# aaletov/open-pcc-metric

Measured on AMD Instinct MI355X. Metric: Mpoints/s for symmetric D1+D2 PSNR, N_ref=N_deg=1M, higher is better.
Workload: dtype f64

## Files before the change

### open_pcc_metric_amd/csrc/pccm_brick.h

```cpp
#pragma once
#include "pccm_grid.h"

namespace pccm {

constexpr int kBXMax = 64;
constexpr int kLcsPitch = kBXMax + 3;
typedef float v2f __attribute__((ext_vector_type(2)));
constexpr float kBigF = 3.0e38f;
constexpr int kExtra = 21;
constexpr float kFar = 1.0e18f;

struct BrickParams {
    int bx;
    int nbx, nby, nbz;
    int64_t per_job;
    uint32_t total;
    int cap;
    unsigned long long *stamps;
    float h32[3], face_lo[3], face_hi[3];
    float org32x, invh32x;
};

__device__ __forceinline__ float face32(float q, int c, int dim, float h, float flo, float fhi)
{
    const float cf = (float)c;
    const float lo = q - __builtin_fmaf(cf, h, flo), hi = __builtin_fmaf(cf, h, fhi) - q;
    const float a = c >= 2 ? lo : INFINITY, b = c <= dim - 3 ? hi : INFINITY;
    return a < b ? a : b;
}

__device__ __forceinline__ float umin_f(float a, float b)
{
    const uint32_t x = __float_as_uint(a), y = __float_as_uint(b);
    return __uint_as_float(x < y ? x : y);
}

constexpr int kPlaneSmall = 2176, kPlaneMid = 3008, kPlaneLarge = 3584;

}
```

### open_pcc_metric_amd/csrc/pccm_brick.hip

```cpp
#include "pccm_brick.h"
#include "pccm_tail_wave.h"

namespace pccm {

#define BRICK_STAMP(k)                                                                       \
    do {                                                                                     \
        if (STAMP) {                                                                         \
            const unsigned long long now_ = __builtin_amdgcn_s_memtime();                    \
            t_sum[k] += now_ - t_last;         \
            t_last = now_;                                                                   \
        }                                                                                    \
    } while (0)

__device__ __forceinline__ void load_normal(const NNOut &o, int row, double &a, double &b, double &c)
{
    if (o.nrm32) {
        const float4 t = o.nrm32[row];
        a = (double)t.x; b = (double)t.y; c = (double)t.z;
    } else {
        const double *np = o.nrm + 3 * (int64_t)row;
        a = np[0]; b = np[1]; c = np[2];
    }
}

__device__ __forceinline__ void tail_append(const QueryJobs &jobs, const QueryJob &J, const float4 q)
{
    const uint32_t pos = atomicAdd(&J.counters[1], 1u);
    reinterpret_cast<float4 *>(J.tail)[pos] = q;
    if (J.blk_cnt) {
        const uint32_t blk = (uint32_t)(__float_as_int(q.w) - (int)J.row_base) >> kTailBlockShift;
        const uint32_t slot = atomicAdd(&J.blk_cnt[blk], 1u);
        if (slot < (uint32_t)kTailBlockCap) J.blk_list[(size_t)blk * kTailBlockCap + slot] = q;
        else if (jobs.err) atomicOr(jobs.err, kErrTailFiled);
        const float nan = __int_as_float(0x7fc00000);
        store_result_rec(J.out, __float_as_int(q.w), nan, nan, nan, -1);
    }
}

template <bool SELF, int BY, int BZ, bool STAMP, int ABL, bool N32, int PL>
__device__ __forceinline__ void brick_body(const QueryJobs &jobs, const GridGeom &g, const BrickParams &bp, const uint32_t vblock)
{
    if (ABL & 32) return;
    const int NT = (int)blockDim.x;
    unsigned long long t_last = STAMP ? __builtin_amdgcn_s_memtime() : 0ull;
    const unsigned long long t_start = t_last;
    unsigned long long t_sum[6] = {0, 0, 0, 0, 0, 0};
    constexpr int kNRow = BY * BZ;
    constexpr int kNRun = (BY + 2) * (BZ + 2);
    static_assert(kNRun <= 64 && kNRow <= 64, "one wave scans the run / row lengths");
    extern __shared__ __attribute__((aligned(16))) float s_pl[];
    static_assert(8 * PL * 4 / 2 < 65536 && 12 * PL < 65536, "plane offsets are 16-bit immediates");
    __shared__ uint16_t s_lcs[kNRun * kLcsPitch];
    __shared__ uint32_t s_g0[kNRun], s_len[kNRun], s_base[kNRun + 1], s_qg0[kNRow], s_qoff[kNRow + 1];
    float *const s_x = s_pl, *const s_y = s_pl + PL, *const s_z = s_pl + 2 * PL, *const s_r = s_pl + 3 * PL;
    const uint32_t lds0 = (uint32_t)(uintptr_t)s_x;
    const int tid = threadIdx.x, lane = tid & 63;
    const int w = __builtin_amdgcn_readfirstlane(tid >> 6);
    const uint32_t nblk = bp.total, xcd = vblock & 7u, slot = vblock >> 3;
    const uint32_t bq = nblk >> 3, br = nblk & 7u;
    int64_t vb = (int64_t)(xcd < br ? xcd * (bq + 1) : br * (bq + 1) + (xcd - br) * bq) + slot;
    const int jb = (jobs.njobs > 1 && vb >= bp.per_job) ? 1 : 0;
    if (jb) vb -= bp.per_job;
    if (vb >= bp.per_job) return;
    const QueryJob &J = jobs.j[jb];
    const int dimx = g.dim[0], dimy = g.dim[1], dimz = g.dim[2];
    const uint32_t vbu = (uint32_t)vb;
    const uint32_t t_xy = vbu / (uint32_t)bp.nbx;
    const uint32_t t_z = t_xy / (uint32_t)bp.nby;
    const int ibx = (int)(vbu - t_xy * (uint32_t)bp.nbx), iby = (int)(t_xy - t_z * (uint32_t)bp.nby), ibz = (int)t_z;
    const int bx0 = ibx * bp.bx, bx1 = min(bx0 + bp.bx, dimx);
    const int by0 = iby * BY, bz0 = ibz * BZ;
    const int sx0 = max(bx0 - 1, 0), sx1 = min(bx1 + 1, dimx);
    const int ncs = sx1 - sx0;
    const uint32_t *__restrict__ cs = J.cs;
    const uint32_t *__restrict__ qcs = J.qcs;
    const Rec32 *__restrict__ srecs = (const Rec32 *)J.srecs;
    const Rec32 *__restrict__ qbase = (const Rec32 *)J.qbase;

    if (w == 0) {
        uint32_t len = 0, g0 = 0;
        if (lane < kNRun) {
            const int y = by0 - 1 + lane % (BY + 2), z = bz0 - 1 + lane / (BY + 2);
            if (y >= 0 && y < dimy && z >= 0 && z < dimz) {
                const uint32_t rowbase = ((uint32_t)z * dimy + y) * dimx;
                g0 = cs[rowbase + sx0];
                len = cs[rowbase + sx1] - g0;
            }
            s_g0[lane] = g0;
            s_len[lane] = len;
        }
        const uint32_t plen = (len + 1u) & ~1u;
        uint32_t inc = plen;
#pragma unroll
        for (int off = 1; off < 64; off <<= 1) {
            const uint32_t o = __shfl_up(inc, off);
            if (lane >= off) inc += o;
        }
        if (lane < kNRun) s_base[lane] = inc - plen;
        if (lane == kNRun - 1) s_base[kNRun] = inc;
    } else if (w == 1) {
        uint32_t len = 0, q0 = 0;
        if (lane < kNRow) {
            const int y = by0 + lane % BY, z = bz0 + lane / BY;
            if (y < dimy && z < dimz) {
                const uint32_t rowbase = ((uint32_t)z * dimy + y) * dimx;
                q0 = qcs[rowbase + bx0];
                len = qcs[rowbase + bx1] - q0;
            }
            s_qg0[lane] = q0;
        }
        uint32_t inc = len;
#pragma unroll
        for (int off = 1; off < 64; off <<= 1) {
            const uint32_t o = __shfl_up(inc, off);
            if (lane >= off) inc += o;
        }
        if (lane < kNRow) s_qoff[lane] = inc - len;
        if (lane == kNRow - 1) s_qoff[kNRow] = inc;
    }
    __syncthreads();
    BRICK_STAMP(0);
    if (ABL & 16) return;
    const uint32_t T = s_base[kNRun], NQ = s_qoff[kNRow];
    if (NQ == 0) return;

    auto query_row = [&](uint32_t qi) {
        int r = 0;
#pragma unroll
        for (int k = 1; k < kNRow; ++k) r += (qi >= s_qoff[k]) ? 1 : 0;
        return r;
    };
    auto load_query = [&](uint32_t qi, int r) {
        return *reinterpret_cast<const float4 *>(&qbase[s_qg0[r] + (qi - s_qoff[r])]);
    };

    if (T > (uint32_t)bp.cap) {
        for (uint32_t qi = tid; qi < NQ; qi += NT) {
            const float4 q = load_query(qi, query_row(qi));
            tail_append(jobs, J, q);
        }
        return;
    }

    uint32_t qi = tid;
    bool have = qi < NQ;
    int rn = 0;
    float4 qn = make_float4(0.f, 0.f, 0.f, 0.f);
    if (have) rn = query_row(qi);

    const NNOut &out = J.out;
    const bool fuse = out.nrm != nullptr;
    const bool fuse_row = fuse && out.normal_mode == PCCM_NORMAL_ROW;
    double n0 = 0.0, n1 = 0.0, n2 = 0.0;
    float4 nraw = make_float4(0.f, 0.f, 0.f, 0.f);
    const bool defer = out.layout == 1;
    auto gather_row_normal = [&](int row, bool on) {
        if (defer) return;
        if (N32) {
            const float4 *src = on ? out.nrm32 + row : reinterpret_cast<const float4 *>(qbase);
            nraw = *src;
        } else if (on) {
            const double *np = out.nrm + 3 * (int64_t)row;
            n0 = np[0]; n1 = np[1]; n2 = np[2];
        }
    };
    {
        const int nw = NT >> 6;
        for (int r0 = w; r0 < kNRun; r0 += 3 * nw) {
            float4 rec[3], rex;
            uint32_t rb[3], rl[3], rg[3];
#pragma unroll
            for (int u = 0; u < 3; ++u) {
                const int r = r0 + u * nw;
                rb[u] = rl[u] = rg[u] = 0u;
                if (r < kNRun) {
                    rb[u] = (uint32_t)__builtin_amdgcn_readfirstlane((int)s_base[r]);
                    rl[u] = (uint32_t)__builtin_amdgcn_readfirstlane((int)s_len[r]);
                    rg[u] = (uint32_t)__builtin_amdgcn_readfirstlane((int)s_g0[r]);
                }
                rec[u] = make_float4(kFar, kFar, kFar, __int_as_float(-1));
                if (!(ABL & 2) && (uint32_t)lane < rl[u]) rec[u] = *reinterpret_cast<const float4 *>(&srecs[rg[u] + (uint32_t)lane]);
            }
            const int xu = lane / kExtra;
            const uint32_t xp = 64u + (uint32_t)(lane - xu * kExtra);
            const uint32_t xb = xu == 0 ? rb[0] : xu == 1 ? rb[1] : rb[2];
            const uint32_t xl = xu == 0 ? rl[0] : xu == 1 ? rl[1] : xu == 2 ? rl[2] : 0u;
            const uint32_t xg = xu == 0 ? rg[0] : xu == 1 ? rg[1] : rg[2];
            rex = make_float4(kFar, kFar, kFar, __int_as_float(-1));
            if (!(ABL & 2) && xp < xl) rex = *reinterpret_cast<const float4 *>(&srecs[xg + xp]);
            uint32_t v[3][2];
            bool in[3];
#pragma unroll
            for (int u = 0; u < 3; ++u) {
                const int r = r0 + u * nw;
                v[u][0] = v[u][1] = 0u;
                in[u] = false;
                if (r < kNRun) {
                    const int y = by0 - 1 + r % (BY + 2), z = bz0 - 1 + r / (BY + 2);
                    in[u] = y >= 0 && y < dimy && z >= 0 && z < dimz;
                    if (in[u] && !(ABL & 8)) {
                        const uint32_t *src = cs + ((uint32_t)z * dimy + y) * dimx + sx0;
                        if (lane <= ncs) v[u][0] = src[lane];
                        if (lane + 64 <= ncs) v[u][1] = src[lane + 64];
                    }
                }
            }
            if (have && r0 == w) qn = load_query(qi, rn);
#pragma unroll
            for (int u = 0; u < 3; ++u) {
                const uint32_t plen = (rl[u] + 1u) & ~1u;
                if ((uint32_t)lane < plen) {
                    const uint32_t f = rb[u] + (uint32_t)lane;
                    s_x[f] = rec[u].x;
                    s_y[f] = rec[u].y;
                    s_z[f] = rec[u].z;
                    s_r[f] = rec[u].w;
                }
            }
            if (xp < ((xl + 1u) & ~1u)) {
                const uint32_t f = xb + xp;
                s_x[f] = rex.x;
                s_y[f] = rex.y;
                s_z[f] = rex.z;
                s_r[f] = rex.w;
            }
#pragma unroll
            for (int u = 0; u < 3; ++u) {
                const uint32_t plen = (rl[u] + 1u) & ~1u;
                for (uint32_t p = (uint32_t)lane + 64u + (uint32_t)kExtra; p < plen; p += 64u) {
                    float4 t = make_float4(kFar, kFar, kFar, __int_as_float(-1));
                    if (!(ABL & 2) && p < rl[u]) t = *reinterpret_cast<const float4 *>(&srecs[rg[u] + p]);
                    const uint32_t f = rb[u] + p;
                    s_x[f] = t.x;
                    s_y[f] = t.y;
                    s_z[f] = t.z;
                    s_r[f] = t.w;
                }
            }
#pragma unroll
            for (int u = 0; u < 3; ++u) {
                const int r = r0 + u * nw;
                if (r < kNRun) {
                    const uint32_t base = lds0 + 4u * rb[u], rebase = base - 4u * rg[u];
                    if (lane <= ncs) s_lcs[r * kLcsPitch + lane] = (uint16_t)(in[u] ? 4u * v[u][0] + rebase : base);
                    if (lane + 64 <= ncs) s_lcs[r * kLcsPitch + lane + 64] = (uint16_t)(in[u] ? 4u * v[u][1] + rebase : base);
                }
            }
        }
        __builtin_amdgcn_sched_barrier(0);
        gather_row_normal(__float_as_int(qn.w), have && fuse_row);
    }
    BRICK_STAMP(1);
    __syncthreads();
    BRICK_STAMP(2);

    int q_iter = 0;
    while (have) {
        const float4 q = qn;
        const int r = rn;
        const int qrow = __float_as_int(q.w);
        const uint32_t qnext = qi + NT;
        const bool hn = qnext < NQ;
        const double qx = (double)q.x, qy = (double)q.y, qz = (double)q.z;
        const int ly = r % BY, lz = r / BY;
        const int cx = min(max((int)floorf((q.x - bp.org32x) * bp.invh32x), bx0), bx1 - 1);
        const int cy = by0 + ly, cz = bz0 + lz;
        const int ja = max(cx - 1, 0) - sx0, jb2 = min(cx + 2, dimx) - sx0;
        float best = kBigF, second = kBigF;
        uint32_t bestpos = 0xffffffffu;
        const v2f qxx = {q.x, q.x}, qyy = {q.y, q.y}, qzz = {q.z, q.z};
#pragma unroll
        for (int dz = 0; dz < 3; ++dz) {
#pragma unroll
            for (int dy = 0; dy < 3; ++dy) {
                const int run = (lz + dz) * (BY + 2) + (ly + dy);
                const uint32_t fsb = s_lcs[run * kLcsPitch + ja], feb = s_lcs[run * kLcsPitch + jb2];
                if constexpr (ABL != 0) {
                for (uint32_t a = fsb & ~7u, ae = (ABL & 1) ? (fsb < feb ? a + 8u : a) : feb; a < ae; a += 8u) {
                    v2f px, py, pz;
                    asm volatile("ds_read_b64 %0, %3\n\tds_read_b64 %1, %3 offset:%4\n\tds_read_b64 %2, %3 offset:%5\n\ts_waitcnt lgkmcnt(0)"
                                 : "=&v"(px), "=&v"(py), "=&v"(pz)
                                 : "v"(a), "n"(4 * PL), "n"(8 * PL)
                                 : "memory");
                    const v2f dx = qxx - px, dy = qyy - py, dz = qzz - pz;
                    v2f dd = dx * dx;
                    dd = __builtin_elementwise_fma(dy, dy, dd);
                    dd = __builtin_elementwise_fma(dz, dz, dd);
                    const float lo = umin_f(dd.x, dd.y);
                    bestpos = __float_as_uint(lo) < __float_as_uint(best) ? a + 8u : bestpos;
                    second = __builtin_amdgcn_fmed3f(best, second, lo);
                    best = umin_f(best, lo);
                }
                } else {
                    uint32_t a = fsb & ~7u;
                    const uint32_t ae = feb;
                    v2f px, py, pz, pr;
                    if (SELF)
                        asm volatile("ds_read_b64 %0, %4\n\tds_read_b64 %1, %4 offset:%5\n\tds_read_b64 %2, %4 offset:%6\n\tds_read_b64 %3, %4 offset:%7"
                                     : "=v"(px), "=v"(py), "=v"(pz), "=v"(pr) : "v"(a), "n"(4 * PL), "n"(8 * PL), "n"(12 * PL) : "memory");
                    else
                        asm volatile("ds_read_b64 %0, %3\n\tds_read_b64 %1, %3 offset:%4\n\tds_read_b64 %2, %3 offset:%5"
                                     : "=v"(px), "=v"(py), "=v"(pz) : "v"(a), "n"(4 * PL), "n"(8 * PL) : "memory");
                    while (a < ae) {
                        if (SELF) asm volatile("s_waitcnt lgkmcnt(0)" : "+v"(px), "+v"(py), "+v"(pz), "+v"(pr) : : "memory");
                        else asm volatile("s_waitcnt lgkmcnt(0)" : "+v"(px), "+v"(py), "+v"(pz) : : "memory");
                        v2f dx = qxx - px, dy = qyy - py, dz = qzz - pz;
                        uint32_t k0 = 0u, k1 = 0u;
                        if (SELF) {
                            k0 = __float_as_int(pr.x) == qrow ? __float_as_uint(kBigF) : 0u;
                            k1 = __float_as_int(pr.y) == qrow ? __float_as_uint(kBigF) : 0u;
                            asm volatile("" : "+v"(k0), "+v"(k1));
                        }
                        asm volatile("" : "+v"(dx), "+v"(dy), "+v"(dz));
                        a += 8u;
                        if (SELF)
                            asm volatile("ds_read_b64 %0, %4\n\tds_read_b64 %1, %4 offset:%5\n\tds_read_b64 %2, %4 offset:%6\n\tds_read_b64 %3, %4 offset:%7"
                                         : "+v"(px), "+v"(py), "+v"(pz), "+v"(pr) : "v"(a), "n"(4 * PL), "n"(8 * PL), "n"(12 * PL) : "memory");
                        else
                            asm volatile("ds_read_b64 %0, %3\n\tds_read_b64 %1, %3 offset:%4\n\tds_read_b64 %2, %3 offset:%5"
                                         : "+v"(px), "+v"(py), "+v"(pz) : "v"(a), "n"(4 * PL), "n"(8 * PL) : "memory");
                        v2f dd = dx * dx;
                        dd = __builtin_elementwise_fma(dy, dy, dd);
                        dd = __builtin_elementwise_fma(dz, dz, dd);
                        float d0 = dd.x, d1 = dd.y;
                        if (SELF) {
                            d0 = __uint_as_float(max(__float_as_uint(d0), k0));
                            d1 = __uint_as_float(max(__float_as_uint(d1), k1));
                        }
                        const float lo = umin_f(d0, d1);
                        bestpos = __float_as_uint(lo) < __float_as_uint(best) ? a : bestpos;
                        second = __builtin_amdgcn_fmed3f(best, second, lo);
                        best = umin_f(best, lo);
                    }
                    if (SELF) asm volatile("s_waitcnt lgkmcnt(0)" : "+v"(px), "+v"(py), "+v"(pz), "+v"(pr) : : "memory");
                    else asm volatile("s_waitcnt lgkmcnt(0)" : "+v"(px), "+v"(py), "+v"(pz) : : "memory");
                }
            }
        }
        BRICK_STAMP(5);
        const float thr = __builtin_fmaf(best, 1.0f + 0x1.0p-18f, 2.0e-36f);
        bool settled = false;
        if (ABL & 4) {
            if (best < 0.0f) store_result(out, qrow, 0.0, 0.0, 0);
            settled = true;
        } else if (bestpos != 0xffffffffu && best < 1.0e30f && second > thr) {
            uint32_t f = (bestpos - 8u - lds0) >> 2;
            float partner;
            {
                const v2f px = *reinterpret_cast<const v2f *>(s_x + f), py = *reinterpret_cast<const v2f *>(s_y + f),
                          pz = *reinterpret_cast<const v2f *>(s_z + f);
                const v2f dx = qxx - px, dy = qyy - py, dz = qzz - pz;
                v2f dd = dx * dx;
                dd = __builtin_elementwise_fma(dy, dy, dd);
                dd = __builtin_elementwise_fma(dz, dz, dd);
                float d0 = dd.x, d1 = dd.y;
                if (SELF) {
                    d0 = (__float_as_int(s_r[f]) == qrow) ? kBigF : d0;
                    d1 = (__float_as_int(s_r[f + 1]) == qrow) ? kBigF : d1;
                }
                const bool first = d0 == best;
                partner = first ? d1 : d0;
                f += first ? 0u : 1u;
            }
            float L = face32(q.x, cx, dimx, bp.h32[0], bp.face_lo[0], bp.face_hi[0]);
            L = fminf(L, face32(q.y, cy, dimy, bp.h32[1], bp.face_lo[1], bp.face_hi[1]));
            L = fminf(L, face32(q.z, cz, dimz, bp.h32[2], bp.face_lo[2], bp.face_hi[2]));
            settled = partner > thr && L > 0.0f && best * 1.00001f < L * L * 0.99999f;
            const float wx = s_x[f], wy = s_y[f], wz = s_z[f];
            const int wrow = __float_as_int(s_r[f]);
            if (settled && defer) {
                store_result_rec(out, qrow, wx, wy, wz, wrow);
            } else if (settled) {
                const double rx = (double)wx, ry = (double)wy, rz = (double)wz;
                const double d64 = gdist64(qx, qy, qz, rx, ry, rz);
                double p = 0.0;
                if (fuse) {
                    double e0 = N32 ? (double)nraw.x : n0, e1 = N32 ? (double)nraw.y : n1, e2 = N32 ? (double)nraw.z : n2;
                    if (!fuse_row) {
                        load_normal(out, wrow, e0, e1, e2);
                    }
                    const double ex = __dsub_rn(qx, rx), ey = __dsub_rn(qy, ry), ez = __dsub_rn(qz, rz);
                    p = __dmul_rn(ex, e0);
                    p = __fma_rn(ey, e1, p);
                    p = __fma_rn(ez, e2, p);
                }
                store_result(out, qrow, d64, p, wrow);
            }
        }
        if (!settled) tail_append(jobs, J, q);
        if (hn) {
            rn = query_row(qnext);
            qn = load_query(qnext, rn);
            gather_row_normal(__float_as_int(qn.w), fuse_row);
        }
        qi = qnext;
        have = hn;
        if (STAMP) {
            BRICK_STAMP(q_iter == 0 ? 3 : 4);
            ++q_iter;
        }
    }
    if (STAMP && lane == 0) {
        unsigned long long *slot = bp.stamps + ((size_t)blockIdx.x * (NT >> 6) + w) * 8;
#pragma unroll
        for (int k = 0; k < 6; ++k) slot[k] = t_sum[k];
        slot[6] = t_start;
        slot[7] = __builtin_amdgcn_s_memtime();
    }
}

template <bool SELF, int BY, int BZ, int PL, bool STAMP = false, int ABL = 0, bool N32 = true>
__global__ __launch_bounds__(1024, 8) void k_brick_query(QueryJobs jobs, GridGeom g, BrickParams bp)
{
    brick_body<SELF, BY, BZ, STAMP, ABL, N32, PL>(jobs, g, bp, blockIdx.x);
}

template <int BY, int BZ, int PL>
__global__ __launch_bounds__(1024) void k_brick_query_free(QueryJobs jobs, GridGeom g, BrickParams bp)
{
    brick_body<false, BY, BZ, false, 0, false, PL>(jobs, g, bp, blockIdx.x);
}

struct BrickShape {
    int by, bz, nt;
};

static BrickShape brick_shape()
{
    static const BrickShape s = [] {
        BrickShape v = {4, 2, 0};
        const char *e = getenv("PCCM_BRICK");
        if (e) {
            int a = 0, b = 0, c = 0;
            const int got = sscanf(e, "%d,%d,%d", &a, &b, &c);
            if (got >= 2) v = {a, b, got == 3 ? c : 0};
        }
        return v;
    }();
    return s;
}

template <int BY, int BZ, int PL>
static void launch_plane(pccm_ctx *ctx, const QueryJobs &jobs, const GridGeom &g, bool self, BrickParams bp, double density_q, int force_nt)
{
    constexpr int kStatic = (BY + 2) * (BZ + 2) * (kLcsPitch * 2 + 12) + (BY * BZ) * 8 + 64;
    static_assert(4 * PL * (int)sizeof(float) + kStatic <= 64 * 1024, "static + dynamic LDS of one workgroup stay under 64 KB");
    const double eq = (double)(BY * BZ) * bp.bx * density_q;
    int nt = ((int)(eq + 2.5 * sqrt(eq)) + 63) / 64 * 64;
    const size_t lds = (size_t)4 * PL * sizeof(float);
    const size_t lds_wg = lds + (size_t)((BY + 2) * (BZ + 2)) * (kLcsPitch * 2 + 16) + 256;
    const int wgs_per_cu = (int)((size_t)160 * 1024 / lds_wg) > 0 ? (int)((size_t)160 * 1024 / lds_wg) : 1;
    const int nt_cap = 64 * (32 / (wgs_per_cu > 16 ? 16 : wgs_per_cu));
    if (nt > nt_cap) nt = nt_cap;
    if (force_nt > 0) nt = force_nt / 64 * 64;
    if (nt < 128) nt = 128;
    if (nt > 1024) nt = 1024;
    bp.total = (uint32_t)(bp.per_job * jobs.njobs);
    dim3 grid(bp.total);
    bp.stamps = nullptr;
#ifdef PCCM_DIAG
    static const bool stamp = [] { const char *e = getenv("PCCM_BRICK_STAMP"); return e && e[0] == '1'; }();
    if (stamp && !self && !ctx->capturing) {
        static unsigned long long *dev = nullptr;
        static size_t dev_slots = 0;
        const size_t slots = (size_t)bp.total * (size_t)(nt >> 6);
        if (slots > dev_slots) {
            if (dev) (void)hipFree(dev);
            dev = nullptr;
            if (hipMalloc((void **)&dev, slots * 8 * sizeof(unsigned long long)) == hipSuccess) dev_slots = slots;
            else dev_slots = 0;
        }
        if (dev) {
            (void)hipMemsetAsync(dev, 0, slots * 8 * sizeof(unsigned long long), ctx->stream);
            bp.stamps = dev;
            PCCM_LAUNCH(ctx, (k_brick_query<false, BY, BZ, PL, true>), grid, dim3(nt), lds, ctx->stream, jobs, g, bp);
            std::vector<unsigned long long> h(slots * 8);
            (void)hipMemcpyAsync(h.data(), dev, h.size() * sizeof(unsigned long long), hipMemcpyDeviceToHost, ctx->stream);
            (void)hipStreamSynchronize(ctx->stream);
            double sum[6] = {0, 0, 0, 0, 0, 0}, life = 0.0;
            unsigned long long first = ~0ull, last = 0ull;
            size_t waves = 0;
            for (size_t i = 0; i < slots; ++i) {
                const unsigned long long *r = &h[i * 8];
                if (r[7] == 0) continue;
                ++waves;
                for (int k = 0; k < 6; ++k) sum[k] += (double)r[k];
                life += (double)(r[7] - r[6]);
                first = r[6] < first ? r[6] : first;
                last = r[7] > last ? r[7] : last;
            }
            const double w = waves ? (double)waves : 1.0;
            fprintf(stderr, "[pccm] brick stamps (s_memtime ticks per wave, %zu waves, nt %d, cap %d): lifetime %.0f, first start -> last end %.0f | "
                            "bounds+barrier %.0f | staging %.0f | barrier %.0f | scan %.0f | epilogue %.0f | leftovers %.0f\n",
                    waves, nt, bp.cap, life / w, (double)(last - first), sum[0] / w, sum[1] / w, sum[2] / w, sum[5] / w, sum[3] / w, sum[4] / w);
            return;
        }
    }
    static const int ablate = [] { const char *e = getenv("PCCM_BRICK_ABLATE"); return e ? atoi(e) : 0; }();
    if (ablate && !self && BY == 4 && BZ == 2) {
        if (ablate == 1) PCCM_LAUNCH(ctx, (k_brick_query<false, 4, 2, PL, false, 1>), grid, dim3(nt), lds, ctx->stream, jobs, g, bp);
        else if (ablate == 2) PCCM_LAUNCH(ctx, (k_brick_query<false, 4, 2, PL, false, 2>), grid, dim3(nt), lds, ctx->stream, jobs, g, bp);
        else if (ablate == 4) PCCM_LAUNCH(ctx, (k_brick_query<false, 4, 2, PL, false, 4>), grid, dim3(nt), lds, ctx->stream, jobs, g, bp);
        else if (ablate == 8) PCCM_LAUNCH(ctx, (k_brick_query<false, 4, 2, PL, false, 8>), grid, dim3(nt), lds, ctx->stream, jobs, g, bp);
        else if (ablate == 16) PCCM_LAUNCH(ctx, (k_brick_query<false, 4, 2, PL, false, 16>), grid, dim3(nt), lds, ctx->stream, jobs, g, bp);
        else if (ablate == 32) PCCM_LAUNCH(ctx, (k_brick_query<false, 4, 2, PL, false, 32>), grid, dim3(nt), lds, ctx->stream, jobs, g, bp);
        else PCCM_LAUNCH(ctx, (k_brick_query<false, 4, 2, PL, false, 15>), grid, dim3(nt), lds, ctx->stream, jobs, g, bp);
        return;
    }
#endif
    static const bool v_free = [] { const char *e = PCCM_DIAG_ENV("PCCM_BRICK_V64"); return e && e[0] == '0'; }();
    if (v_free && !self) {
        PCCM_LAUNCH(ctx, (k_brick_query_free<BY, BZ, PL>), grid, dim3(nt), lds, ctx->stream, jobs, g, bp);
        return;
    }
    bool n32 = true;
    for (int k = 0; k < jobs.njobs; ++k) n32 = n32 && (jobs.j[k].out.nrm == nullptr || jobs.j[k].out.nrm32 != nullptr);
    if (self) PCCM_LAUNCH(ctx, (k_brick_query<true, BY, BZ, PL>), grid, dim3(nt), lds, ctx->stream, jobs, g, bp);
    else if (n32) PCCM_LAUNCH(ctx, (k_brick_query<false, BY, BZ, PL, false, 0, true>), grid, dim3(nt), lds, ctx->stream, jobs, g, bp);
    else PCCM_LAUNCH(ctx, (k_brick_query<false, BY, BZ, PL, false, 0, false>), grid, dim3(nt), lds, ctx->stream, jobs, g, bp);
}

template <int BY, int BZ>
static void launch_shape(pccm_ctx *ctx, const QueryJobs &jobs, const GridGeom &g, bool self, BrickParams bp, double density_s,
                         double density_q, int force_nt)
{
    bp.nby = (g.dim[1] + BY - 1) / BY;
    bp.nbz = (g.dim[2] + BZ - 1) / BZ;
    bp.per_job = (int64_t)bp.nbx * bp.nby * bp.nbz;
    const double expect = (double)((BY + 2) * (BZ + 2)) * (bp.bx + 2) * density_s;
    const double margin = fmin(0.25 * expect, 8.0 * sqrt(expect));
    int cap = (int)(expect + margin) + 64;
    static const int cap_env = [] { const char *e = getenv("PCCM_BRICK_CAP"); return e ? atoi(e) : 0; }();
    if (cap_env > 0) cap = cap_env;
    if (cap < 256) cap = 256;
    if (cap + 4 <= kPlaneSmall) {
        bp.cap = kPlaneSmall - 4;
        launch_plane<BY, BZ, kPlaneSmall>(ctx, jobs, g, self, bp, density_q, force_nt);
    } else if (cap + 4 <= kPlaneMid) {
        bp.cap = kPlaneMid - 4;
        launch_plane<BY, BZ, kPlaneMid>(ctx, jobs, g, self, bp, density_q, force_nt);
    } else {
        bp.cap = kPlaneLarge - 4;
        launch_plane<BY, BZ, kPlaneLarge>(ctx, jobs, g, self, bp, density_q, force_nt);
    }
}

int launch_brick_query(pccm_ctx *ctx, const QueryJobs &jobs, const GridGeom &g, bool self)
{
    BrickParams bp;
    static const int bx_env = [] { const char *e = PCCM_DIAG_ENV("PCCM_BRICK_BX"); return e ? atoi(e) : 0; }();
    const int bx_max = bx_env > 0 ? bx_env : 48;
    const int nbx = (g.dim[0] + bx_max - 1) / bx_max;
    bp.bx = (g.dim[0] + nbx - 1) / nbx;
    if (bp.bx > kBXMax) bp.bx = kBXMax;
    bp.nbx = (g.dim[0] + bp.bx - 1) / bp.bx;
    bp.nby = bp.nbz = 0;
    bp.per_job = 0;
    bp.total = 0;
    bp.cap = 0;
    bp.stamps = nullptr;
    for (int a = 0; a < 3; ++a) {
        const double top = g.org[a] + (double)g.dim[a] * g.h[a];
        const double M = fmax(fabs(g.org[a]), fabs(top)) + 2.0 * g.h[a];
        const double slack = g.slack[a] + 8.0 * M * 0x1.0p-24;
        bp.h32[a] = (float)g.h[a];
        if (a == 0) {
            bp.org32x = (float)g.org[0];
            bp.invh32x = (float)g.inv_h[0];
        }
        bp.face_lo[a] = (float)(g.org[a] - g.h[a] + slack);
        bp.face_hi[a] = (float)(g.org[a] + 2.0 * g.h[a] - slack);
    }
    const Grid &gr = ctx->grid;
    const int64_t nmax = gr.n[0] > gr.n[1] ? gr.n[0] : gr.n[1];
    const double density = gr.ncells > 0 ? (double)nmax / (double)gr.ncells : 1.5;
    int64_t nqmax = 0;
    for (int k = 0; k < jobs.njobs; ++k) nqmax = jobs.j[k].nq > nqmax ? jobs.j[k].nq : nqmax;
    const double density_q = gr.ncells > 0 ? (double)nqmax / (double)gr.ncells : 1.5;
    BrickShape sh = brick_shape();
    static const bool shape_forced = getenv("PCCM_BRICK") != nullptr;
    if (!shape_forced && density_q <= 0.55 * density) sh = {4, 4, 0};
    if (sh.by == 2 && sh.bz == 2) launch_shape<2, 2>(ctx, jobs, g, self, bp, density, density_q, sh.nt);
    else if (sh.by == 4 && sh.bz == 4) launch_shape<4, 4>(ctx, jobs, g, self, bp, density, density_q, sh.nt);
    else launch_shape<4, 2>(ctx, jobs, g, self, bp, density, density_q, sh.nt);
    PCCM_HIP(hipGetLastError());
    return PCCM_OK;
}

}
```

Before: 11160.

## Pad brick LDS runs so each window scan does fixed unrolled trips

Pads every staged run in LDS by a fixed number of far-away sentinel pairs so each 3x3 neighbour window can run a fixed count of fully unrolled, software-pipelined trips. LDS reads for the next trip are issued while the current distance math runs. Windows longer than the fixed trips are finished in a tail loop driven by a bitmask. The cost is extra LDS footprint and wasted distance work on the padding sentinels, and padding is skipped when the brick would exceed the cap.

Measured after the change: 10890. -2.4%, worse.

```diff
diff --git a/open_pcc_metric_amd/csrc/pccm_brick.h b/open_pcc_metric_amd/csrc/pccm_brick.h
--- a/open_pcc_metric_amd/csrc/pccm_brick.h
+++ b/open_pcc_metric_amd/csrc/pccm_brick.h
@@ -9,6 +9,10 @@
 constexpr float kBigF = 3.0e38f;
 constexpr int kExtra = 21;
 constexpr float kFar = 1.0e18f;
+#ifndef PCCM_BRICK_EVEN_TRIPS
+#define PCCM_BRICK_EVEN_TRIPS 3
+#endif
+constexpr int kEvenTrips = PCCM_BRICK_EVEN_TRIPS;
 
 struct BrickParams {
     int bx;
@@ -16,6 +20,7 @@
     int64_t per_job;
     uint32_t total;
     int cap;
+    int even;
     unsigned long long *stamps;
     float h32[3], face_lo[3], face_hi[3];
     float org32x, invh32x;
diff --git a/open_pcc_metric_amd/csrc/pccm_brick.hip b/open_pcc_metric_amd/csrc/pccm_brick.hip
--- a/open_pcc_metric_amd/csrc/pccm_brick.hip
+++ b/open_pcc_metric_amd/csrc/pccm_brick.hip
@@ -35,6 +35,31 @@
         const float nan = __int_as_float(0x7fc00000);
         store_result_rec(J.out, __float_as_int(q.w), nan, nan, nan, -1);
     }
+}
+
+template <bool SELF, int PL, int OFF, bool FIRST>
+__device__ __forceinline__ void scan_issue(v2f &px, v2f &py, v2f &pz, v2f &pr, const uint32_t a)
+{
+    static_assert(12 * PL + OFF < 65536, "plane offsets are 16-bit immediates");
+    if constexpr (SELF && FIRST)
+        asm volatile("ds_read_b64 %0, %4 offset:%5\n\tds_read_b64 %1, %4 offset:%6\n\tds_read_b64 %2, %4 offset:%7\n\tds_read_b64 %3, %4 offset:%8"
+                     : "=v"(px), "=v"(py), "=v"(pz), "=v"(pr) : "v"(a), "n"(OFF), "n"(4 * PL + OFF), "n"(8 * PL + OFF), "n"(12 * PL + OFF) : "memory");
+    else if constexpr (SELF)
+        asm volatile("ds_read_b64 %0, %4 offset:%5\n\tds_read_b64 %1, %4 offset:%6\n\tds_read_b64 %2, %4 offset:%7\n\tds_read_b64 %3, %4 offset:%8"
+                     : "+v"(px), "+v"(py), "+v"(pz), "+v"(pr) : "v"(a), "n"(OFF), "n"(4 * PL + OFF), "n"(8 * PL + OFF), "n"(12 * PL + OFF) : "memory");
+    else if constexpr (FIRST)
+        asm volatile("ds_read_b64 %0, %3 offset:%4\n\tds_read_b64 %1, %3 offset:%5\n\tds_read_b64 %2, %3 offset:%6"
+                     : "=v"(px), "=v"(py), "=v"(pz) : "v"(a), "n"(OFF), "n"(4 * PL + OFF), "n"(8 * PL + OFF) : "memory");
+    else
+        asm volatile("ds_read_b64 %0, %3 offset:%4\n\tds_read_b64 %1, %3 offset:%5\n\tds_read_b64 %2, %3 offset:%6"
+                     : "+v"(px), "+v"(py), "+v"(pz) : "v"(a), "n"(OFF), "n"(4 * PL + OFF), "n"(8 * PL + OFF) : "memory");
+}
+
+template <bool SELF>
+__device__ __forceinline__ void scan_wait(v2f &px, v2f &py, v2f &pz, v2f &pr)
+{
+    if constexpr (SELF) asm volatile("s_waitcnt lgkmcnt(0)" : "+v"(px), "+v"(py), "+v"(pz), "+v"(pr) : : "memory");
+    else asm volatile("s_waitcnt lgkmcnt(0)" : "+v"(px), "+v"(py), "+v"(pz) : : "memory");
 }
 
 template <bool SELF, int BY, int BZ, bool STAMP, int ABL, bool N32, int PL>
@@ -96,8 +121,10 @@
             const uint32_t o = __shfl_up(inc, off);
             if (lane >= off) inc += o;
         }
-        if (lane < kNRun) s_base[lane] = inc - plen;
-        if (lane == kNRun - 1) s_base[kNRun] = inc;
+        const uint32_t tot = (uint32_t)__builtin_amdgcn_readlane((int)inc, kNRun - 1);
+        const uint32_t padn = (ABL == 0 && (bp.even & 1) && tot + (uint32_t)(kNRun * 2 * kEvenTrips) <= (uint32_t)bp.cap) ? 2u * kEvenTrips : 0u;
+        if (lane < kNRun) s_base[lane] = inc - plen + (uint32_t)lane * padn;
+        if (lane == kNRun - 1) s_base[kNRun] = tot | (padn ? 0x80000000u : 0u);
     } else if (w == 1) {
         uint32_t len = 0, q0 = 0;
         if (lane < kNRow) {
@@ -121,7 +148,10 @@
     __syncthreads();
     BRICK_STAMP(0);
     if (ABL & 16) return;
-    const uint32_t T = s_base[kNRun], NQ = s_qoff[kNRow];
+    const uint32_t Traw = (uint32_t)__builtin_amdgcn_readfirstlane((int)s_base[kNRun]), NQ = s_qoff[kNRow];
+    const uint32_t T = Traw & 0x7fffffffu;
+    const bool even = (Traw >> 31) != 0u;
+    const uint32_t padn = even ? 2u * kEvenTrips : 0u;
     if (NQ == 0) return;
 
     auto query_row = [&](uint32_t qi) {
@@ -168,15 +198,16 @@
         const int nw = NT >> 6;
         for (int r0 = w; r0 < kNRun; r0 += 3 * nw) {
             float4 rec[3], rex;
-            uint32_t rb[3], rl[3], rg[3];
+            uint32_t rb[3], rl[3], rg[3], rq[3];
 #pragma unroll
             for (int u = 0; u < 3; ++u) {
                 const int r = r0 + u * nw;
-                rb[u] = rl[u] = rg[u] = 0u;
+                rb[u] = rl[u] = rg[u] = rq[u] = 0u;
                 if (r < kNRun) {
                     rb[u] = (uint32_t)__builtin_amdgcn_readfirstlane((int)s_base[r]);
                     rl[u] = (uint32_t)__builtin_amdgcn_readfirstlane((int)s_len[r]);
                     rg[u] = (uint32_t)__builtin_amdgcn_readfirstlane((int)s_g0[r]);
+                    rq[u] = padn;
                 }
                 rec[u] = make_float4(kFar, kFar, kFar, __int_as_float(-1));
                 if (!(ABL & 2) && (uint32_t)lane < rl[u]) rec[u] = *reinterpret_cast<const float4 *>(&srecs[rg[u] + (uint32_t)lane]);
@@ -186,6 +217,7 @@
             const uint32_t xb = xu == 0 ? rb[0] : xu == 1 ? rb[1] : rb[2];
             const uint32_t xl = xu == 0 ? rl[0] : xu == 1 ? rl[1] : xu == 2 ? rl[2] : 0u;
             const uint32_t xg = xu == 0 ? rg[0] : xu == 1 ? rg[1] : rg[2];
+            const uint32_t xq = xu == 0 ? rq[0] : xu == 1 ? rq[1] : xu == 2 ? rq[2] : 0u;
             rex = make_float4(kFar, kFar, kFar, __int_as_float(-1));
             if (!(ABL & 2) && xp < xl) rex = *reinterpret_cast<const float4 *>(&srecs[xg + xp]);
             uint32_t v[3][2];
@@ -208,7 +240,7 @@
             if (have && r0 == w) qn = load_query(qi, rn);
 #pragma unroll
             for (int u = 0; u < 3; ++u) {
-                const uint32_t plen = (rl[u] + 1u) & ~1u;
+                const uint32_t plen = ((rl[u] + 1u) & ~1u) + rq[u];
                 if ((uint32_t)lane < plen) {
                     const uint32_t f = rb[u] + (uint32_t)lane;
                     s_x[f] = rec[u].x;
@@ -217,7 +249,7 @@
                     s_r[f] = rec[u].w;
                 }
             }
-            if (xp < ((xl + 1u) & ~1u)) {
+            if (xp < ((xl + 1u) & ~1u) + xq) {
                 const uint32_t f = xb + xp;
                 s_x[f] = rex.x;
                 s_y[f] = rex.y;
@@ -226,7 +258,7 @@
             }
 #pragma unroll
             for (int u = 0; u < 3; ++u) {
-                const uint32_t plen = (rl[u] + 1u) & ~1u;
+                const uint32_t plen = ((rl[u] + 1u) & ~1u) + rq[u];
                 for (uint32_t p = (uint32_t)lane + 64u + (uint32_t)kExtra; p < plen; p += 64u) {
                     float4 t = make_float4(kFar, kFar, kFar, __int_as_float(-1));
                     if (!(ABL & 2) && p < rl[u]) t = *reinterpret_cast<const float4 *>(&srecs[rg[u] + p]);
@@ -269,6 +301,99 @@
         float best = kBigF, second = kBigF;
         uint32_t bestpos = 0xffffffffu;
         const v2f qxx = {q.x, q.x}, qyy = {q.y, q.y}, qzz = {q.z, q.z};
+        if (ABL == 0 && even) {
+            uint32_t over = 0u;
+            auto trip = [&](auto kc, const uint32_t a, v2f &px, v2f &py, v2f &pz, v2f &pr) {
+                constexpr int k = decltype(kc)::value;
+                __builtin_amdgcn_sched_barrier(0);
+                scan_wait<SELF>(px, py, pz, pr);
+                v2f dx = qxx - px, dy = qyy - py, dz = qzz - pz;
+                uint32_t k0 = 0u, k1 = 0u;
+                if (SELF) {
+                    k0 = __float_as_int(pr.x) == qrow ? __float_as_uint(kBigF) : 0u;
+                    k1 = __float_as_int(pr.y) == qrow ? __float_as_uint(kBigF) : 0u;
+                    asm volatile("" : "+v"(k0), "+v"(k1));
+                }
+                asm volatile("" : "+v"(dx), "+v"(dy), "+v"(dz));
+                if constexpr (k + 1 < kEvenTrips) scan_issue<SELF, PL, 8 * (k + 1), false>(px, py, pz, pr, a);
+                v2f dd = dx * dx;
+                dd = __builtin_elementwise_fma(dy, dy, dd);
+                dd = __builtin_elementwise_fma(dz, dz, dd);
+                float d0 = dd.x, d1 = dd.y;
+                if (SELF) {
+                    d0 = __uint_as_float(max(__float_as_uint(d0), k0));
+                    d1 = __uint_as_float(max(__float_as_uint(d1), k1));
+                }
+                const float lo = umin_f(d0, d1);
+                bestpos = __float_as_uint(lo) < __float_as_uint(best) ? a + 8u * (uint32_t)(k + 1) : bestpos;
+                second = __builtin_amdgcn_fmed3f(best, second, lo);
+                best = umin_f(best, lo);
+            };
+#pragma unroll
+            for (int dz = 0; dz < 3; ++dz) {
+#pragma unroll
+                for (int dy = 0; dy < 3; ++dy) {
+                    const int run = (lz + dz) * (BY + 2) + (ly + dy);
+                    const uint32_t fsb = s_lcs[run * kLcsPitch + ja], feb = s_lcs[run * kLcsPitch + jb2];
+                    const uint32_t a = fsb & ~7u;
+                    v2f px, py, pz, pr;
+                    scan_issue<SELF, PL, 0, true>(px, py, pz, pr, a);
+                    trip(std::integral_constant<int, 0>{}, a, px, py, pz, pr);
+                    if constexpr (kEvenTrips > 1) trip(std::integral_constant<int, 1>{}, a, px, py, pz, pr);
+                    if constexpr (kEvenTrips > 2) trip(std::integral_constant<int, 2>{}, a, px, py, pz, pr);
+                    if constexpr (kEvenTrips > 3) trip(std::integral_constant<int, 3>{}, a, px, py, pz, pr);
+                    static_assert(kEvenTrips >= 1 && kEvenTrips <= 4, "trips are written out");
+                    over |= a + 8u * kEvenTrips < feb ? 1u << (dz * 3 + dy) : 0u;
+                }
+            }
+            if (over) {
+                uint32_t a = 0u, ae = 0u;
+                auto next_window = [&]() {
+                    const uint32_t w9 = (uint32_t)__builtin_ctz(over);
+                    over &= over - 1u;
+                    const uint32_t wz = (w9 * 11u) >> 5, wy = w9 - 3u * wz;
+                    const uint32_t run = ((uint32_t)lz + wz) * (BY + 2) + (uint32_t)ly + wy;
+                    a = (s_lcs[run * kLcsPitch + ja] & ~7u) + 8u * kEvenTrips;
+                    ae = s_lcs[run * kLcsPitch + jb2];
+                };
+                next_window();
+                v2f px, py, pz, pr;
+                scan_issue<SELF, PL, 0, true>(px, py, pz, pr, a);
+                for (;;) {
+                    scan_wait<SELF>(px, py, pz, pr);
+                    v2f dx = qxx - px, dy = qyy - py, dz = qzz - pz;
+                    uint32_t k0 = 0u, k1 = 0u;
+                    if (SELF) {
+                        k0 = __float_as_int(pr.x) == qrow ? __float_as_uint(kBigF) : 0u;
+                        k1 = __float_as_int(pr.y) == qrow ? __float_as_uint(kBigF) : 0u;
+                        asm volatile("" : "+v"(k0), "+v"(k1));
+                    }
+                    asm volatile("" : "+v"(dx), "+v"(dy), "+v"(dz));
+                    a += 8u;
+                    const uint32_t apos = a;
+                    bool last = false;
+                    if (a >= ae) {
+                        if (over) next_window();
+                        else last = true;
+                    }
+                    scan_issue<SELF, PL, 0, false>(px, py, pz, pr, a);
+                    v2f dd = dx * dx;
+                    dd = __builtin_elementwise_fma(dy, dy, dd);
+                    dd = __builtin_elementwise_fma(dz, dz, dd);
+                    float d0 = dd.x, d1 = dd.y;
+                    if (SELF) {
+                        d0 = __uint_as_float(max(__float_as_uint(d0), k0));
+                        d1 = __uint_as_float(max(__float_as_uint(d1), k1));
+                    }
+                    const float lo = umin_f(d0, d1);
+                    bestpos = __float_as_uint(lo) < __float_as_uint(best) ? apos : bestpos;
+                    second = __builtin_amdgcn_fmed3f(best, second, lo);
+                    best = umin_f(best, lo);
+                    if (last) break;
+                }
+                scan_wait<SELF>(px, py, pz, pr);
+            }
+        } else {
 #pragma unroll
         for (int dz = 0; dz < 3; ++dz) {
 #pragma unroll
@@ -337,6 +462,7 @@
                 }
             }
         }
+        }
         BRICK_STAMP(5);
         const float thr = __builtin_fmaf(best, 1.0f + 0x1.0p-18f, 2.0e-36f);
         bool settled = false;
@@ -559,6 +685,10 @@
     bp.total = 0;
     bp.cap = 0;
     bp.stamps = nullptr;
+    {
+        const char *e = getenv("PCCM_BRICK_EVEN");
+        bp.even = e ? atoi(e) : 1;
+    }
     for (int a = 0; a < 3; ++a) {
         const double top = g.org[a] + (double)g.dim[a] * g.h[a];
         const double M = fmax(fabs(g.org[a]), fabs(top)) + 2.0 * g.h[a];
```
